# ml4ai/mliis

Hardware: AMD Instinct MI355X
Metric: inner-loop images/sec (EfficientLab-6-3, 224x224, 5-shot) (higher is better)
Workload: dtype f32 (the long-K decoder convs and their filter gradients with every operand split exactly into three bf16 terms on the matrix cores, 6 term products, f32 accumulate: fp32-equivalent products; everything else the fp32 instruction)

## Files before the change

mliis_amd/csrc/mbconv_small.hip:

```cpp
#include "common.hpp"

namespace mliis {

constexpr int kSmThreads = 512;
constexpr int kSmWaves = kSmThreads / 64;
constexpr int kSmMaxPix = 2048;

struct SmallGeom {
  int N, H, W, C, HS, nitems, npix;
};

template <int V>
struct SmV {
  float v[V];
};
#define SMV_FOR _Pragma("unroll") for (int i = 0; i < V; ++i)
template <int V> __device__ __forceinline__ SmV<V> vzero() { SmV<V> r; SMV_FOR r.v[i] = 0.f; return r; }
template <int V> __device__ __forceinline__ SmV<V> vfill(float x) { SmV<V> r; SMV_FOR r.v[i] = x; return r; }
template <int V> __device__ __forceinline__ SmV<V> vadd(SmV<V> a, SmV<V> b) { SMV_FOR a.v[i] += b.v[i]; return a; }
template <int V> __device__ __forceinline__ SmV<V> vsub(SmV<V> a, SmV<V> b) { SMV_FOR a.v[i] -= b.v[i]; return a; }
template <int V> __device__ __forceinline__ SmV<V> vmul(SmV<V> a, SmV<V> b) { SMV_FOR a.v[i] *= b.v[i]; return a; }
template <int V> __device__ __forceinline__ SmV<V> vscale(SmV<V> a, float s) { SMV_FOR a.v[i] *= s; return a; }
template <int V> __device__ __forceinline__ SmV<V> vfma(SmV<V> a, SmV<V> b, SmV<V> c) { SMV_FOR c.v[i] = fmaf(a.v[i], b.v[i], c.v[i]); return c; }
template <int V> __device__ __forceinline__ SmV<V> vswish(SmV<V> a) { SMV_FOR a.v[i] = swish_f(a.v[i]); return a; }
template <int V> __device__ __forceinline__ SmV<V> vswish_grad(SmV<V> a) { SMV_FOR a.v[i] = swish_grad_f(a.v[i]); return a; }
template <int V> __device__ __forceinline__ SmV<V> vxhat(SmV<V> x, SmV<V> m, SmV<V> r) { SMV_FOR x.v[i] = (x.v[i] - m.v[i]) * r.v[i]; return x; }
template <int V> __device__ __forceinline__ SmV<V> vaffine(SmV<V> xh, SmV<V> g, SmV<V> b) { SMV_FOR xh.v[i] = fmaf(xh.v[i], g.v[i], b.v[i]); return xh; }
template <int V> __device__ __forceinline__ SmV<V> vbn_dx(SmV<V> g, SmV<V> xh, SmV<V> a, SmV<V> b, SmV<V> ga, SmV<V> rs) {
  SMV_FOR g.v[i] = ga.v[i] * rs.v[i] * (g.v[i] - a.v[i] - xh.v[i] * b.v[i]);
  return g;
}
template <int V> __device__ __forceinline__ SmV<V> vld(const float* __restrict__ p) { SmV<V> r; SMV_FOR r.v[i] = p[i]; return r; }
template <int V> __device__ __forceinline__ void vst(float* __restrict__ p, SmV<V> a) { SMV_FOR p[i] = a.v[i]; }

template <int V> struct SmSlot { static constexpr int F = V; };
template <int V> __device__ __forceinline__ SmV<V> lds_ld(const float* __restrict__ base, int slot) {
  SmV<V> r;
  if constexpr (V == 2) {
    const float2 t = *reinterpret_cast<const float2*>(base + slot * 2);
    r.v[0] = t.x; r.v[1] = t.y;
  } else {
    const float4 t = *reinterpret_cast<const float4*>(base + slot * 4);
    r.v[0] = t.x; r.v[1] = t.y; r.v[2] = t.z; r.v[V - 1] = t.w;
  }
  return r;
}
template <int V> __device__ __forceinline__ void lds_st(float* __restrict__ base, int slot, SmV<V> a) {
  if constexpr (V == 2) {
    *reinterpret_cast<float2*>(base + slot * 2) = make_float2(a.v[0], a.v[1]);
  } else {
    *reinterpret_cast<float4*>(base + slot * 4) = make_float4(a.v[0], a.v[1], a.v[2], a.v[V - 1]);
  }
}

template <int V> struct SmRun { static constexpr int R = 32 / V; };
template <int V>
__device__ __forceinline__ int sm_channel_group(int C) {
  constexpr int R = SmRun<V>::R;
  const int G = C / V, runs = (G + R - 1) / R;
  const int b = blockIdx.x, xcd = b & 7, j = b >> 3;
  const int run = (j / R) * 8 + xcd, sub = j % R;
  if (run >= runs) return -1;
  const int gq = run * R + sub;
  return gq < G ? gq : -1;
}
static inline int sm_grid(int C, int V) {
  const int R = 32 / V, G = C / V, runs = (G + R - 1) / R;
  return ((runs + 7) / 8) * 8 * R;
}
static inline int sm_group_width(int C, int k, int cus) { return (k == 5 && C % 2 == 0 && C / 2 <= cus) ? 2 : 4; }

template <int CTRL, int ROW_MASK>
__device__ __forceinline__ float sm_dpp_add(float v) {
  return v + __builtin_bit_cast(float, __builtin_amdgcn_update_dpp(0, __builtin_bit_cast(int, v), CTRL, ROW_MASK, 0xF, true));
}
__device__ __forceinline__ float sm_wave_sum63(float v) {
  v = sm_dpp_add<0xB1, 0xF>(v);
  v = sm_dpp_add<0x4E, 0xF>(v);
  v = sm_dpp_add<0x141, 0xF>(v);
  v = sm_dpp_add<0x140, 0xF>(v);
  v = sm_dpp_add<0x142, 0xA>(v);
  v = sm_dpp_add<0x143, 0xC>(v);
  return v;
}
template <int V> __device__ __forceinline__ SmV<V> sm_wave_sum63(SmV<V> a) { SMV_FOR a.v[i] = sm_wave_sum63(a.v[i]); return a; }

__device__ __forceinline__ void sm_lds_barrier() {
  __builtin_amdgcn_fence(__ATOMIC_RELEASE, "workgroup", "local");
  __builtin_amdgcn_s_barrier();
  __builtin_amdgcn_fence(__ATOMIC_ACQUIRE, "workgroup", "local");
}

template <int V>
__device__ __forceinline__ void sm_block_sum2(SmV<V>& a, SmV<V>& b, float* red) {
  const int t = threadIdx.x, lane = t & 63, wave = t >> 6;
  const SmV<V> wa = sm_wave_sum63(a), wb = sm_wave_sum63(b);
  if (lane == 63) {
    SMV_FOR {
      red[(wave * 2 + 0) * 4 + i] = wa.v[i];
      red[(wave * 2 + 1) * 4 + i] = wb.v[i];
    }
  }
  sm_lds_barrier();
  if (t < 8) {
    float sacc = red[t];
#pragma unroll
    for (int w = 1; w < kSmWaves; ++w) sacc += red[w * 8 + t];
    red[kSmWaves * 8 + t] = sacc;
  }
  sm_lds_barrier();
  SMV_FOR {
    a.v[i] = red[kSmWaves * 8 + i];
    b.v[i] = red[kSmWaves * 8 + 4 + i];
  }
}

typedef unsigned sm_u32x4 __attribute__((ext_vector_type(4)));
typedef unsigned sm_u32x2 __attribute__((ext_vector_type(2)));
constexpr unsigned kSmOob = 0xFFFFFFF0u;
__device__ __forceinline__ __amdgpu_buffer_rsrc_t sm_rsrc(const void* p) {
  return __builtin_amdgcn_make_buffer_rsrc(const_cast<void*>(p), 0, 0x80000000u, 0x00020000);
}
template <int V, typename T = float>
__device__ __forceinline__ SmV<V> sm_ld(__amdgpu_buffer_rsrc_t r, unsigned off) {
  SmV<V> o;
  if constexpr (sizeof(T) == 2 && V == 2) {
    const unsigned u = __builtin_amdgcn_raw_buffer_load_b32(r, (int)off, 0, 0);
    o.v[0] = __uint_as_float(u << 16); o.v[1] = __uint_as_float(u & 0xffff0000u);
  } else if constexpr (sizeof(T) == 2) {
    const sm_u32x2 u = __builtin_amdgcn_raw_buffer_load_b64(r, (int)off, 0, 0);
    o.v[0] = __uint_as_float(u.x << 16); o.v[1] = __uint_as_float(u.x & 0xffff0000u);
    o.v[2] = __uint_as_float(u.y << 16); o.v[V - 1] = __uint_as_float(u.y & 0xffff0000u);
  } else if constexpr (V == 2) {
    const sm_u32x2 u = __builtin_amdgcn_raw_buffer_load_b64(r, (int)off, 0, 0);
    o.v[0] = __uint_as_float(u.x); o.v[1] = __uint_as_float(u.y);
  } else {
    const sm_u32x4 u = __builtin_amdgcn_raw_buffer_load_b128(r, (int)off, 0, 0);
    o.v[0] = __uint_as_float(u.x); o.v[1] = __uint_as_float(u.y); o.v[2] = __uint_as_float(u.z); o.v[3] = __uint_as_float(u.w);
  }
  return o;
}
template <int V, typename T = float>
__device__ __forceinline__ void sm_st(__amdgpu_buffer_rsrc_t r, unsigned off, SmV<V> a) {
  if constexpr (sizeof(T) == 2 && V == 2) {
    __builtin_amdgcn_raw_buffer_store_b32(pack_bf16_pair(a.v[0], a.v[1]), r, (int)off, 0, 0);
  } else if constexpr (sizeof(T) == 2) {
    sm_u32x2 u;
    u.x = pack_bf16_pair(a.v[0], a.v[1]); u.y = pack_bf16_pair(a.v[2], a.v[V - 1]);
    __builtin_amdgcn_raw_buffer_store_b64(u, r, (int)off, 0, 0);
  } else if constexpr (V == 2) {
    sm_u32x2 u;
    u.x = __float_as_uint(a.v[0]); u.y = __float_as_uint(a.v[1]);
    __builtin_amdgcn_raw_buffer_store_b64(u, r, (int)off, 0, 0);
  } else {
    sm_u32x4 u;
    u.x = __float_as_uint(a.v[0]); u.y = __float_as_uint(a.v[1]); u.z = __float_as_uint(a.v[2]); u.w = __float_as_uint(a.v[V - 1]);
    __builtin_amdgcn_raw_buffer_store_b128(u, r, (int)off, 0, 0);
  }
}

template <int V, typename T> __device__ __forceinline__ SmV<V> sm_stored(SmV<V> a) {
  if constexpr (sizeof(T) == 2) {
#pragma unroll
    for (int i = 0; i < V; ++i) a.v[i] = bf16_round_f(a.v[i]);
  }
  return a;
}

struct SmStrip {
  bool act;
  int n, h0, w;
  unsigned off0, rstride;
  int H;
  __device__ __forceinline__ unsigned poff(int j) const { return (act && h0 + j < H) ? off0 + (unsigned)j * rstride : kSmOob; }
  unsigned boff0, brow;
  __device__ __forceinline__ unsigned bpoff(int j) const { return (act && h0 + j < H) ? boff0 + (unsigned)j * brow : kSmOob; }
  __device__ __forceinline__ bool ok(int j) const { return act && h0 + j < H; }
};
__device__ __forceinline__ SmStrip sm_strip(const SmallGeom& g, int c, int esize = 4, int V = 4) {
  SmStrip s;
  const int pl = threadIdx.x;
  s.act = pl < g.nitems;
  int w_ = 0, hs = 0, n = 0;
  if (s.act) {
    w_ = pl % g.W;
    const int r = pl / g.W;
    hs = r % g.HS;
    n = r / g.HS;
  }
  s.n = n;
  s.h0 = hs * 4;
  s.w = w_;
  s.H = g.H;
  s.off0 = (unsigned)((((n * g.H + s.h0) * g.W + w_) * g.C + c) * esize);
  s.rstride = (unsigned)(g.W * g.C * esize);
  s.boff0 = (unsigned)((((c / V) * g.npix + (n * g.H + s.h0) * g.W + w_) * V) * esize);
  s.brow = (unsigned)(g.W * V * esize);
  return s;
}

struct SmallFwd {
  const float* z0;
  const float* part0;
  int nblk0;
  const float *gamma0, *beta0;
  float *mean0, *rstd0, *mm0, *mv0;
  const float* w;
  const float *gamma1, *beta1;
  float *mean1, *rstd1, *mm1, *mv1;
  float* a0;
  float* z1;
  float* a1;
  float* s;
  float* z0b;
  int z1_blocked;
  SmallGeom g;
  float eps, one_minus_momentum;
};

template <int K, int V> struct SmTapsInRegs { static constexpr bool value = K == 3 || V <= 2; };

template <int K, int V, typename T = float>
__global__ __launch_bounds__(kSmThreads) void mbconv_dw_fwd_small_k(SmallFwd p) {
  extern __shared__ __attribute__((aligned(16))) float smem[];
  typedef SmV<V> VT;
  constexpr int F = SmSlot<V>::F;
  const SmallGeom g = p.g;
  float* tileA = smem;
  float* wl = tileA + (size_t)g.npix * F;
  float* red = wl + K * K * F;
  float* pool = red + (kSmWaves + 1) * 2 * 4;
  double* fold = reinterpret_cast<double*>(pool + kSmThreads * F);
  float* stat = reinterpret_cast<float*>(fold + 8);
  const int cq = sm_channel_group<V>(g.C);
  if (cq < 0) return;
  const int t = threadIdx.x, lane = t & 63, wave = t >> 6;
  const int c = cq * V;
  const SmStrip st = sm_strip(g, c, (int)sizeof(T), V);
// ... 55 lines not shown
  VT acc[4];
#pragma unroll
  for (int j = 0; j < 4; ++j) acc[j] = vzero<V>();
  if (st.act) {
    const float* imgA = tileA + (size_t)st.n * g.H * g.W * F;
    if constexpr (SmTapsInRegs<K, V>::value) {
      VT wreg[K * K];
#pragma unroll
      for (int i = 0; i < K * K; ++i) wreg[i] = lds_ld<V>(wl, i);
#pragma unroll
      for (int r = 0; r < K + 3; ++r) {
        const int hi = st.h0 - P + r;
        const bool rok = (unsigned)hi < (unsigned)g.H;
        VT row[K];
#pragma unroll
        for (int kx = 0; kx < K; ++kx) {
          const int wi = st.w - P + kx;
          row[kx] = (rok && (unsigned)wi < (unsigned)g.W) ? lds_ld<V>(imgA, hi * g.W + wi) : vzero<V>();
        }
#pragma unroll
        for (int j = 0; j < 4; ++j) {
          const int ky = r - j;
          if (ky >= 0 && ky < K) {
#pragma unroll
            for (int kx = 0; kx < K; ++kx) acc[j] = vfma(row[kx], wreg[ky * K + kx], acc[j]);
          }
        }
        if (K == 5) __builtin_amdgcn_sched_barrier(0);
      }
    } else {
#pragma unroll 1
      for (int r = 0; r < K + 3; ++r) {
        const int hi = st.h0 - P + r;
        const bool rok = (unsigned)hi < (unsigned)g.H;
        VT row[K];
#pragma unroll
        for (int kx = 0; kx < K; ++kx) {
          const int wi = st.w - P + kx;
          row[kx] = (rok && (unsigned)wi < (unsigned)g.W) ? lds_ld<V>(imgA, hi * g.W + wi) : vzero<V>();
        }
#pragma unroll
        for (int j = 0; j < 4; ++j) {
          const int ky = r - j;
          if (ky >= 0 && ky < K) {
#pragma unroll
            for (int kx = 0; kx < K; ++kx) acc[j] = vfma(row[kx], lds_ld<V>(wl, ky * K + kx), acc[j]);
          }
        }
      }
    }
  }
  {
    const __amdgpu_buffer_rsrc_t rz1 = sm_rsrc(p.z1);
#pragma unroll
    for (int j = 0; j < 4; ++j) {
      acc[j] = sm_stored<V, T>(acc[j]);
      sm_st<V, T>(rz1, p.z1_blocked ? st.bpoff(j) : st.poff(j), acc[j]);
    }
  }
  VT s1 = vzero<V>(), s2 = vzero<V>();
#pragma unroll
  for (int j = 0; j < 4; ++j)
    if (st.ok(j)) s1 = vadd(s1, acc[j]);
  sm_block_sum2<V>(s1, s2, red);
  const float inv_n = 1.0f / (float)g.npix;
  const VT m1 = vscale(s1, inv_n);
  VT d2 = vzero<V>(), dummy = vzero<V>();
#pragma unroll
  for (int j = 0; j < 4; ++j)
    if (st.ok(j)) {
      const VT d = vsub(acc[j], m1);
      d2 = vfma(d, d, d2);
    }
  sm_block_sum2<V>(d2, dummy, red);
  const VT var1 = vscale(d2, inv_n);
  VT r1;
  SMV_FOR r1.v[i] = 1.0f / sqrtf(var1.v[i] + p.eps);
  VT a1v[4];
  {
    const VT ga = vld<V>(p.gamma1 + c), be = vld<V>(p.beta1 + c);
    VT ps = vzero<V>();
#pragma unroll
    for (int j = 0; j < 4; ++j) {
      a1v[j] = sm_stored<V, T>(vswish(vaffine(vxhat(acc[j], m1, r1), ga, be)));
      if (st.ok(j)) ps = vadd(ps, a1v[j]);
    }
    lds_st<V>(pool, t, ps);
    const __amdgpu_buffer_rsrc_t ra1 = sm_rsrc(p.a1);
#pragma unroll
    for (int j = 0; j < 4; ++j) sm_st<V, T>(ra1, st.poff(j), a1v[j]);
  }
  sm_lds_barrier();
  {
    const int per = g.HS * g.W;
    for (int img = wave; img < g.N; img += kSmWaves) {
      VT a = vzero<V>();
      for (int i = lane; i < per; i += 64) a = vadd(a, lds_ld<V>(pool, img * per + i));
      a = sm_wave_sum63(a);
      if (lane == 63) vst<V>(p.s + (long long)img * g.C + c, vscale(a, 1.0f / (float)(g.H * g.W)));
    }
  }
  if (t < V) {
    const float mf = stat[t], vf = stat[8 + t];
    p.mean0[c + t] = mf;
    p.rstd0[c + t] = stat[4 + t];
    if (p.mm0 != nullptr) {
      p.mm0[c + t] = mmv0 - (mmv0 - mf) * p.one_minus_momentum;
      p.mv0[c + t] = mvv0 - (mvv0 - vf) * p.one_minus_momentum;
    }
    float m1t = 0.f, r1t = 0.f, v1t = 0.f;
    SMV_FOR if (i == t) {
      m1t = m1.v[i];
      r1t = r1.v[i];
      v1t = var1.v[i];
    }
    p.mean1[c + t] = m1t;
    p.rstd1[c + t] = r1t;
    if (p.mm1 != nullptr) {
      p.mm1[c + t] = mmv1 - (mmv1 - m1t) * p.one_minus_momentum;
      p.mv1[c + t] = mvv1 - (mvv1 - v1t) * p.one_minus_momentum;
    }
  }
}

struct SmallBwd {
  const float* da2;
  const float* gate;
  const float* chan_add;
  const float* z1;
  const float *mean1, *rstd1, *gamma1, *beta1;
  const float* w;
  const float* z0;
  const float *mean0, *rstd0, *gamma0, *beta0;
  float *dgamma1, *dbeta1, *dw, *dgamma0, *dbeta0;
  float* dz0;
  const float* z0b;
  int z1_blocked;
  SmallGeom g;
};

template <int K, int V, typename T = float>
__global__ __launch_bounds__(kSmThreads) void mbconv_dw_bwd_small_k(SmallBwd p) {
  extern __shared__ __attribute__((aligned(16))) float smem[];
  typedef SmV<V> VT;
  constexpr int F = SmSlot<V>::F;
  const SmallGeom g = p.g;
  float* tileA = smem;
  float* tileD = tileA + (size_t)g.npix * F;
  float* wl = tileD + (size_t)g.npix * F;
  float* red = wl + K * K * F;
  float* wred = red + (kSmWaves + 1) * 2 * 4;
  constexpr bool PARK = K == 5 && V == 4;
  float* tileX = wred + kSmWaves * K * K * F;
  const int cq = sm_channel_group<V>(g.C);
  if (cq < 0) return;
  const int t = threadIdx.x, lane = t & 63, wave = t >> 6;
  const int c = cq * V;
  const SmStrip st = sm_strip(g, c, (int)sizeof(T), V);
  const float inv_n = 1.0f / (float)g.npix;
  VT zv[4], dv[4], z0v[4];
  {
    const bool zb = p.z0b != nullptr;
    const __amdgpu_buffer_rsrc_t rz1 = sm_rsrc(p.z1), rd = sm_rsrc(p.da2), rz0 = sm_rsrc(zb ? p.z0b : p.z0);
#pragma unroll
    for (int j = 0; j < 4; ++j) {
      zv[j] = sm_ld<V, T>(rz1, (p.z1_blocked & 1) ? st.bpoff(j) : st.poff(j));
      dv[j] = sm_ld<V, T>(rd, (p.z1_blocked & 2) ? st.bpoff(j) : st.poff(j));
      z0v[j] = sm_ld<V, T>(rz0, zb ? st.bpoff(j) : st.poff(j));
    }
  }
  if (t < K * K) lds_st<V>(wl, t, vld<V>(p.w + (long long)t * g.C + c));
  VT gt = vfill<V>(1.f), ca = vzero<V>();
  if (st.act && p.gate != nullptr) gt = vld<V>(p.gate + (long long)st.n * g.C + c);
  if (st.act && p.chan_add != nullptr) ca = vld<V>(p.chan_add + (long long)st.n * g.C + c);
  const VT m0 = vld<V>(p.mean0 + c), r0_ = vld<V>(p.rstd0 + c), ga0_ = vld<V>(p.gamma0 + c), be0_ = vld<V>(p.beta0 + c);
  {
    const VT m1 = vld<V>(p.mean1 + c), r1 = vld<V>(p.rstd1 + c), ga = vld<V>(p.gamma1 + c), be = vld<V>(p.beta1 + c);
    VT s1 = vzero<V>(), s2 = vzero<V>();
#pragma unroll
    for (int j = 0; j < 4; ++j) {
      const VT xh = vxhat(zv[j], m1, r1);
      VT gg = vmul(vfma(dv[j], gt, ca), vswish_grad(vaffine(xh, ga, be)));
      if (!st.ok(j)) gg = vzero<V>();
      zv[j] = xh;
      dv[j] = gg;
      s1 = vadd(s1, gg);
      s2 = vfma(gg, xh, s2);
    }
    sm_block_sum2<V>(s1, s2, red);
    if (t == 0) {
      vst<V>(p.dbeta1 + c, s1);
      vst<V>(p.dgamma1 + c, s2);
    }
    const VT a = vscale(s1, inv_n), b = vscale(s2, inv_n);
#pragma unroll
    for (int j = 0; j < 4; ++j) {
      const VT d = vbn_dx(dv[j], zv[j], a, b, ga, r1);
      dv[j] = st.ok(j) ? d : vzero<V>();
      if (st.ok(j)) lds_st<V>(tileD, (st.n * g.H + st.h0 + j) * g.W + st.w, d);
    }
  }
#pragma unroll
  for (int j = 0; j < 4; ++j) {
    const VT xh = vxhat(z0v[j], m0, r0_);
    z0v[j] = xh;
    if (st.ok(j)) lds_st<V>(tileA, (st.n * g.H + st.h0 + j) * g.W + st.w, vswish(vaffine(xh, ga0_, be0_)));
    if (PARK && st.ok(j)) lds_st<V>(tileX, (st.n * g.H + st.h0 + j) * g.W + st.w, xh);
  }
  __syncthreads();
  constexpr int P = (K - 1) / 2;
  {
    VT wacc[K * K];
#pragma unroll
    for (int i = 0; i < K * K; ++i) wacc[i] = vzero<V>();
    if (st.act) {
      const float* imgA = tileA + (size_t)st.n * g.H * g.W * F;
#pragma unroll
      for (int r = 0; r < K + 3; ++r) {
        const int hi = st.h0 - P + r;
        const bool rok = (unsigned)hi < (unsigned)g.H;
        VT row[K];
#pragma unroll
        for (int kx = 0; kx < K; ++kx) {
          const int wi = st.w - P + kx;
          row[kx] = (rok && (unsigned)wi < (unsigned)g.W) ? lds_ld<V>(imgA, hi * g.W + wi) : vzero<V>();
        }
#pragma unroll
        for (int j = 0; j < 4; ++j) {
          const int ky = r - j;
          if (ky >= 0 && ky < K) {
#pragma unroll
            for (int kx = 0; kx < K; ++kx) wacc[ky * K + kx] = vfma(row[kx], dv[j], wacc[ky * K + kx]);
          }
        }
        if (K == 5) __builtin_amdgcn_sched_barrier(0);
      }
    }
#pragma unroll
    for (int i = 0; i < K * K; ++i) {
      const VT v = sm_wave_sum63(wacc[i]);
      if (lane == 63) lds_st<V>(wred, wave * (K * K) + i, v);
    }
  }
  __builtin_amdgcn_sched_barrier(0);
  VT acc[4];
#pragma unroll
  for (int j = 0; j < 4; ++j) acc[j] = vzero<V>();
  if (st.act) {
    const float* imgD = tileD + (size_t)st.n * g.H * g.W * F;
    constexpr bool REGS = SmTapsInRegs<K, V>::value;
    VT wreg[REGS ? K * K : 1];
    if constexpr (REGS) {
#pragma unroll
      for (int i = 0; i < K * K; ++i) wreg[i] = lds_ld<V>(wl, i);
    }
    auto body = [&](int r) {
      const int hi = st.h0 - P + r;
      const bool rok = (unsigned)hi < (unsigned)g.H;
      VT row[K];
#pragma unroll
      for (int x = 0; x < K; ++x) {
        const int wi = st.w - P + x;
        row[x] = (rok && (unsigned)wi < (unsigned)g.W) ? lds_ld<V>(imgD, hi * g.W + wi) : vzero<V>();
      }
#pragma unroll
      for (int j = 0; j < 4; ++j) {
        const int ky = (K - 1) - (r - j);
        if (ky >= 0 && ky < K) {
#pragma unroll
          for (int x = 0; x < K; ++x) {
            const VT wv = REGS ? wreg[REGS ? ky * K + (K - 1 - x) : 0] : lds_ld<V>(wl, ky * K + (K - 1 - x));
            acc[j] = vfma(row[x], wv, acc[j]);
          }
        }
      }
    };
    if constexpr (REGS) {
#pragma unroll
      for (int r = 0; r < K + 3; ++r) {
        body(r);
        if (K == 5) __builtin_amdgcn_sched_barrier(0);
      }
    } else {
#pragma unroll 1
      for (int r = 0; r < K + 3; ++r) body(r);
    }
  }
  __syncthreads();
  if (t < K * K) {
    VT v = lds_ld<V>(wred, t);
#pragma unroll
    for (int wv = 1; wv < kSmWaves; ++wv) v = vadd(v, lds_ld<V>(wred, wv * (K * K) + t));
    vst<V>(p.dw + (long long)t * g.C + c, v);
  }
  {
    VT ga0 = ga0_, be0 = be0_, r0 = r0_;
    if constexpr (PARK) {
      const float* pg = p.gamma0 + c;
      const float* pb = p.beta0 + c;
      const float* pr = p.rstd0 + c;
      asm volatile("" : "+v"(pg), "+v"(pb), "+v"(pr));
      ga0 = vld<V>(pg);
      be0 = vld<V>(pb);
      r0 = vld<V>(pr);
#pragma unroll
      for (int j = 0; j < 4; ++j) z0v[j] = st.ok(j) ? lds_ld<V>(tileX, (st.n * g.H + st.h0 + j) * g.W + st.w) : vzero<V>();
    }
    VT s1 = vzero<V>(), s2 = vzero<V>();
#pragma unroll
    for (int j = 0; j < 4; ++j) {
      VT gg = vmul(acc[j], vswish_grad(vaffine(z0v[j], ga0, be0)));
      if (!st.ok(j)) gg = vzero<V>();
      acc[j] = gg;
      s1 = vadd(s1, gg);
      s2 = vfma(gg, z0v[j], s2);
    }
    sm_block_sum2<V>(s1, s2, red);
    if (t == 0) {
      vst<V>(p.dbeta0 + c, s1);
      vst<V>(p.dgamma0 + c, s2);
    }
    const VT a = vscale(s1, inv_n), b = vscale(s2, inv_n);
    const __amdgpu_buffer_rsrc_t rdz = sm_rsrc(p.dz0);
#pragma unroll
    for (int j = 0; j < 4; ++j)
      if (st.ok(j)) sm_st<V, T>(rdz, st.poff(j), vbn_dx(acc[j], z0v[j], a, b, ga0, r0));
  }
}
#undef SMV_FOR

static bool small_geom(int N, int H, int W, int C, int k, int stride, SmallGeom* g) {
  if (N <= 0 || H <= 0 || W <= 0 || C <= 0 || (C & 3) || stride != 1 || (k != 3 && k != 5)) return false;
  const long long npix = (long long)N * H * W;
  const int HS = (H + 3) / 4;
  const long long nitems = (long long)N * HS * W;
  if (npix > kSmMaxPix || nitems > kSmThreads || npix * C * 4 >= (1LL << 31)) return false;
  *g = SmallGeom{N, H, W, C, HS, (int)nitems, (int)npix};
  return true;
}
static size_t small_fwd_lds(const SmallGeom& g, int k) {
  return ((size_t)g.npix + (size_t)k * k + (kSmWaves + 1) * 2 + kSmThreads) * 16 + 8 * 8 + 16 * 4;
}
static size_t small_bwd_lds(const SmallGeom& g, int k) { return ((size_t)g.npix * (k == 5 ? 3 : 2) + (size_t)k * k + (kSmWaves + 1) * 2 + (size_t)kSmWaves * k * k) * 16; }

template <typename Kern>
static int small_attr(Kern kern, size_t lds_max, int* done) {
  if (*done) return MLIIS_OK;
  hipError_t e = hipFuncSetAttribute(reinterpret_cast<const void*>(kern), hipFuncAttributeMaxDynamicSharedMemorySize, (int)lds_max);
  if (e != hipSuccess) return set_error(MLIIS_ERR_LAUNCH, "mbconv_small: cannot reserve %zu bytes of LDS: %s", lds_max, hipGetErrorString(e));
  *done = 1;
  return MLIIS_OK;
}
static int sm_num_cus() {
  static int cus = 0;
  if (cus == 0) {
    int dev = 0;
    hipDeviceProp_t prop;
    cus = (hipGetDevice(&dev) == hipSuccess && hipGetDeviceProperties(&prop, dev) == hipSuccess && prop.multiProcessorCount > 0)
              ? prop.multiProcessorCount : 256;
  }
  return cus;
}
static SmallGeom small_max_geom() { return SmallGeom{1, 1, 1, 4, 1, kSmThreads, kSmMaxPix}; }

template <int K, int V, typename T>
static int small_launch_fwd_t(const SmallFwd& p, int C, size_t lds, hipStream_t stream) {
  static int attr = 0;
  int rc;
  if ((rc = small_attr(mbconv_dw_fwd_small_k<K, V, T>, small_fwd_lds(small_max_geom(), K), &attr))) return rc;
  hipLaunchKernelGGL((mbconv_dw_fwd_small_k<K, V, T>), dim3(sm_grid(C, V)), dim3(kSmThreads), lds, stream, p);
  return MLIIS_OK;
}
template <int K, int V>
static int small_launch_fwd(const SmallFwd& p, int C, size_t lds, int dt, hipStream_t stream) {
  return dt == MLIIS_DT_BF16 ? small_launch_fwd_t<K, V, bf16s>(p, C, lds, stream) : small_launch_fwd_t<K, V, float>(p, C, lds, stream);
}
template <int K, int V, typename T>
static int small_launch_bwd_t(const SmallBwd& p, int C, size_t lds, hipStream_t stream) {
  static int attr = 0;
  int rc;
  if ((rc = small_attr(mbconv_dw_bwd_small_k<K, V, T>, small_bwd_lds(small_max_geom(), K), &attr))) return rc;
  hipLaunchKernelGGL((mbconv_dw_bwd_small_k<K, V, T>), dim3(sm_grid(C, V)), dim3(kSmThreads), lds, stream, p);
  return MLIIS_OK;
}
template <int K, int V>
static int small_launch_bwd(const SmallBwd& p, int C, size_t lds, int dt, hipStream_t stream) {
  return dt == MLIIS_DT_BF16 ? small_launch_bwd_t<K, V, bf16s>(p, C, lds, stream) : small_launch_bwd_t<K, V, float>(p, C, lds, stream);
}

}

using namespace mliis;

extern "C" {

int mliis_mbconv_dw_small_supported(int N, int H, int W, int C, int k, int stride) {
  SmallGeom g;
  return small_geom(N, H, W, C, k, stride, &g) ? 1 : 0;
}

int mliis_mbconv_dw_small_group_width(int C, int k) { return C > 0 ? sm_group_width(C, k, sm_num_cus()) : 0; }

int mliis_mbconv_dw_fwd_small(const float* z0, const float* part0, int nblk0, const float* gamma0, const float* beta0, float* mean0,
                              float* rstd0, float* moving_mean0, float* moving_var0, const float* w, const float* gamma1, const float* beta1,
                              float* mean1, float* rstd1, float* moving_mean1, float* moving_var1, float* a0, float* z1, float* a1, float* s,
                              int N, int H, int W, int C, int k, float eps, float momentum, int group_width, int act_dtype, float* z0_blocked,
                              int z1_blocked, hipStream_t stream) {
  SmallGeom g;
  MLIIS_REQUIRE(small_geom(N, H, W, C, k, 1, &g), MLIIS_ERR_UNSUPPORTED,
                "mbconv_dw_fwd_small: shape N=%d H=%d W=%d C=%d k=%d is not eligible (mliis_mbconv_dw_small_supported)", N, H, W, C, k);
  MLIIS_REQUIRE(z0 && part0 && nblk0 > 0 && gamma0 && beta0 && mean0 && rstd0 && w && gamma1 && beta1 && mean1 && rstd1 && z1 && a1 && s,
                MLIIS_ERR_ARG, "mbconv_dw_fwd_small: null pointer");
  MLIIS_REQUIRE((moving_mean0 == nullptr) == (moving_var0 == nullptr) && (moving_mean1 == nullptr) == (moving_var1 == nullptr), MLIIS_ERR_ARG,
                "mbconv_dw_fwd_small: moving mean / variance come in pairs");
  MLIIS_REQUIRE(aligned16(z0) && aligned16(part0) && aligned16(gamma0) && aligned16(beta0) && aligned16(mean0) && aligned16(rstd0) &&
                    aligned16(w) && aligned16(gamma1) && aligned16(beta1) && aligned16(mean1) && aligned16(rstd1) && aligned16(a0) &&
                    aligned16(z1) && aligned16(a1) && aligned16(s) && aligned16(moving_mean1) && aligned16(moving_var1),
                MLIIS_ERR_ALIGN, "mbconv_dw_fwd_small: pointers must be 16-byte aligned");
  const int V = group_width ? group_width : sm_group_width(C, k, sm_num_cus());
  MLIIS_REQUIRE((V == 2 || V == 4) && C % V == 0, MLIIS_ERR_ARG, "mbconv_dw_fwd_small: group_width %d must be 0, 2 or 4 and divide C = %d", V, C);
  MLIIS_REQUIRE(aligned16(z0_blocked), MLIIS_ERR_ALIGN, "mbconv_dw_fwd_small: z0_blocked must be 16-byte aligned");
  SmallFwd p{z0, part0, nblk0, gamma0, beta0, mean0, rstd0, moving_mean0, moving_var0, w, gamma1, beta1, mean1, rstd1, moving_mean1,
             moving_var1, a0, z1, a1, s, z0_blocked, z1_blocked, g, eps, 1.0f - momentum};
  const size_t lds = small_fwd_lds(g, k);
  int rc;
  MLIIS_REQUIRE(act_dtype == MLIIS_DT_F32 || act_dtype == MLIIS_DT_BF16, MLIIS_ERR_ARG, "mbconv_dw_fwd_small: bad act_dtype");
  if (k == 3) rc = V == 2 ? small_launch_fwd<3, 2>(p, C, lds, act_dtype, stream) : small_launch_fwd<3, 4>(p, C, lds, act_dtype, stream);
  else rc = V == 2 ? small_launch_fwd<5, 2>(p, C, lds, act_dtype, stream) : small_launch_fwd<5, 4>(p, C, lds, act_dtype, stream);
  if (rc) return rc;
  MLIIS_CHECK_LAUNCH("mbconv_dw_fwd_small");
  return MLIIS_OK;
}

int mliis_mbconv_dw_bwd_small(const float* da2, const float* gate, const float* chan_add, const float* z1, const float* mean1,
                              const float* rstd1, const float* gamma1, const float* beta1, const float* w, const float* z0, const float* mean0,
                              const float* rstd0, const float* gamma0, const float* beta0, float* dgamma1, float* dbeta1, float* dw,
                              float* dgamma0, float* dbeta0, float* dz0, int N, int H, int W, int C, int k, int group_width, int act_dtype,
                              const float* z0_blocked, int z1_blocked, hipStream_t stream) {
  SmallGeom g;
  MLIIS_REQUIRE(small_geom(N, H, W, C, k, 1, &g), MLIIS_ERR_UNSUPPORTED,
                "mbconv_dw_bwd_small: shape N=%d H=%d W=%d C=%d k=%d is not eligible (mliis_mbconv_dw_small_supported)", N, H, W, C, k);
  MLIIS_REQUIRE(da2 && z1 && mean1 && rstd1 && gamma1 && beta1 && w && z0 && mean0 && rstd0 && gamma0 && beta0 && dgamma1 && dbeta1 && dw &&
                    dgamma0 && dbeta0 && dz0,
                MLIIS_ERR_ARG, "mbconv_dw_bwd_small: null pointer");
  MLIIS_REQUIRE(aligned16(da2) && aligned16(gate) && aligned16(chan_add) && aligned16(z1) && aligned16(mean1) && aligned16(rstd1) &&
                    aligned16(gamma1) && aligned16(beta1) && aligned16(w) && aligned16(z0) && aligned16(mean0) && aligned16(rstd0) &&
                    aligned16(gamma0) && aligned16(beta0) && aligned16(dgamma1) && aligned16(dbeta1) && aligned16(dw) && aligned16(dgamma0) &&
                    aligned16(dbeta0) && aligned16(dz0),
                MLIIS_ERR_ALIGN, "mbconv_dw_bwd_small: pointers must be 16-byte aligned");
  const int V = group_width ? group_width : sm_group_width(C, k, sm_num_cus());
  MLIIS_REQUIRE((V == 2 || V == 4) && C % V == 0, MLIIS_ERR_ARG, "mbconv_dw_bwd_small: group_width %d must be 0, 2 or 4 and divide C = %d", V, C);
  MLIIS_REQUIRE(aligned16(z0_blocked), MLIIS_ERR_ALIGN, "mbconv_dw_bwd_small: z0_blocked must be 16-byte aligned");
  SmallBwd p{da2, gate, chan_add, z1, mean1, rstd1, gamma1, beta1, w, z0, mean0, rstd0, gamma0, beta0, dgamma1, dbeta1, dw, dgamma0, dbeta0,
             dz0, z0_blocked, z1_blocked, g};
  const size_t lds = small_bwd_lds(g, k);
  int rc;
  MLIIS_REQUIRE(act_dtype == MLIIS_DT_F32 || act_dtype == MLIIS_DT_BF16, MLIIS_ERR_ARG, "mbconv_dw_bwd_small: bad act_dtype");
  if (k == 3) rc = V == 2 ? small_launch_bwd<3, 2>(p, C, lds, act_dtype, stream) : small_launch_bwd<3, 4>(p, C, lds, act_dtype, stream);
  else rc = V == 2 ? small_launch_bwd<5, 2>(p, C, lds, act_dtype, stream) : small_launch_bwd<5, 4>(p, C, lds, act_dtype, stream);
  if (rc) return rc;
  MLIIS_CHECK_LAUNCH("mbconv_dw_bwd_small");
  return MLIIS_OK;
}
}
```

mliis_amd/csrc/se.hip:

```cpp
#include "common.hpp"
#include "se_wgrad.hpp"

namespace mliis {

constexpr int kMaxR = 128;
constexpr int kSeThreads = 1024;

template <int U>
__device__ __forceinline__ float dot_strided(const float* __restrict__ a, int sa, const float* __restrict__ b, long long sb, int n) {
  float acc = 0.f;
  for (int i = 0; i < n; i += U) {
    float x[U], y[U];
#pragma unroll
    for (int u = 0; u < U; ++u) {
      const int k = i + u < n ? i + u : n - 1;
      x[u] = a[(long long)k * sa];
      y[u] = b[(long long)k * sb];
    }
#pragma unroll
    for (int u = 0; u < U; ++u) acc = fmaf(i + u < n ? x[u] : 0.f, y[u], acc);
  }
  return acc;
}

constexpr int kSeFastDot = 24;
template <bool FAST>
__global__ __launch_bounds__(kSeThreads) void se_mlp_fwd_k(const float* __restrict__ s_part, int chunks, float scale,
                                                    float* __restrict__ s_out, const float* __restrict__ w1,
                                                    const float* __restrict__ b1, const float* __restrict__ w2,
                                                    const float* __restrict__ b2, float* __restrict__ hpre,
                                                    float* __restrict__ gate, int C, int R) {
  __shared__ float sh[kMaxR];
  __shared__ float red[kSeThreads];
  __shared__ float red2[8 * kMaxR];
  extern __shared__ float sn[];
  const int n = blockIdx.x, t = threadIdx.x;
  const int CL = kSeThreads / R;
  const int j = t % R, cl = t / R;
  const int cnt = (cl < CL && cl < C) ? (C - cl + CL - 1) / CL : 0;
  float w1v[FAST ? kSeFastDot : 1], w2v[FAST ? 32 : 1], b1v = 0.f, b2v = 0.f;
  if constexpr (FAST) {
    const int cc = t < C ? t : C - 1;
#pragma unroll
    for (int i = 0; i < kSeFastDot; ++i) w1v[i] = w1[(long long)(cl + (i < cnt ? i : 0) * CL < C ? cl + (i < cnt ? i : 0) * CL : 0) * R + j];
#pragma unroll
    for (int k = 0; k < 32; ++k) w2v[k] = w2[(long long)(k < R ? k : R - 1) * C + cc];
    b1v = b1[t < R ? t : 0];
    b2v = b2[cc];
  }
  for (int c = t; c < C; c += kSeThreads) {
    const float* pp = s_part + ((long long)n * chunks) * C + c;
    float a = 0.f;
    for (int k = 0; k < chunks; k += 8) {
      float v[8];
#pragma unroll
      for (int u = 0; u < 8; ++u) v[u] = pp[(long long)(k + u < chunks ? k + u : chunks - 1) * C];
#pragma unroll
      for (int u = 0; u < 8; ++u) a += k + u < chunks ? v[u] : 0.f;
    }
    a *= scale;
    sn[c] = a;
    if (s_out != nullptr) s_out[(long long)n * C + c] = a;
  }
  __syncthreads();
  float part = 0.f;
  if constexpr (FAST) {
#pragma unroll
    for (int i = 0; i < kSeFastDot; ++i) part = fmaf(i < cnt ? sn[cl + i * CL] : 0.f, w1v[i], part);
  } else {
    if (cnt > 0) part = dot_strided<8>(sn + cl, CL, w1 + (long long)cl * R + j, (long long)CL * R, cnt);
  }
  red[t] = part;
  __syncthreads();
  if (t < 8 * R) {
    const int g = t / R;
    float h = 0.f;
    for (int k = g; k < CL; k += 8) h += red[k * R + j];
    red2[g * R + j] = h;
  }
  __syncthreads();
  if (t < R) {
    float h = FAST ? b1v : b1[t];
#pragma unroll
    for (int g = 0; g < 8; ++g) h += red2[g * R + t];
    hpre[(long long)n * R + t] = h;
    sh[t] = swish_f(h);
  }
  __syncthreads();
  if constexpr (FAST) {
    if (t < C) {
      float a = b2v;
#pragma unroll
      for (int k = 0; k < 32; ++k) a = fmaf(k < R ? sh[k] : 0.f, w2v[k], a);
      gate[(long long)n * C + t] = sigmoid_f(a);
    }
    return;
  }
  for (int c = t; c < C; c += kSeThreads) {
    float a = b2[c];
    for (int k = 0; k < R; k += 8) {
      float wv[8];
#pragma unroll
      for (int u = 0; u < 8; ++u) wv[u] = w2[(long long)(k + u < R ? k + u : R - 1) * C + c];
#pragma unroll
      for (int u = 0; u < 8; ++u) a = fmaf(k + u < R ? sh[k + u] : 0.f, wv[u], a);
    }
    gate[(long long)n * C + c] = sigmoid_f(a);
  }
}

template <bool FAST>
__global__ __launch_bounds__(kSeThreads) void se_mlp_bwd_k(const float* __restrict__ dgate, int dgate_groups, int HW,
                                                    const float* __restrict__ gate,
                                                    const float* __restrict__ hpre, const float* __restrict__ w1,
                                                    const float* __restrict__ w1t,
                                                    const float* __restrict__ w2, float* __restrict__ dpre2,
                                                    float* __restrict__ dpre1, float* __restrict__ chan_add, int C, int R,
                                                    float inv_hw, const float* __restrict__ sums, int sums_nblk,
                                                    float* __restrict__ stage1) {
  __shared__ float sd1[kMaxR];
  extern __shared__ float sd2[];
  const int n = blockIdx.x, t = threadIdx.x, lane = t & 63, wave = t >> 6;
  float* d2 = dpre2 + (long long)n * C;
  const int g_lo = dgate_groups > 0 ? (n * HW) / 16 : 0, g_hi = dgate_groups > 0 ? ((n + 1) * HW - 1) / 16 : -1;
  if constexpr (FAST) {
    const int cc = t < C ? t : C - 1;
    const float gte = gate[(long long)n * C + cc];
    float w2v[2][16], w1v[32], hp[2];
#pragma unroll
    for (int r = 0; r < 2; ++r) {
      const int jj = wave + 16 * r < R ? wave + 16 * r : R - 1;
      hp[r] = hpre[(long long)n * R + jj];
#pragma unroll
      for (int u = 0; u < 16; ++u) w2v[r][u] = w2[(long long)jj * C + (lane + 64 * u < C ? lane + 64 * u : C - 1)];
    }
#pragma unroll
    for (int k = 0; k < 32; ++k) {
      const int kk = k < R ? k : R - 1;
      w1v[k] = w1t != nullptr ? w1t[(long long)kk * C + cc] : w1[(long long)cc * R + kk];
    }
    float dg = 0.f;
    if (sums != nullptr) {
      const int G = kSeThreads / C;
      const int g = t / C, c = t - g * C;
      float* scr = sd2 + 5 * C;
      if (g < G) {
        float p[5] = {0.f, 0.f, 0.f, 0.f, 0.f};
        const float* base = sums + ((long long)n * sums_nblk) * 5 * C + c;
        for (int b = g; b < sums_nblk; b += 4 * G) {
          float v[4][5];
#pragma unroll
          for (int u = 0; u < 4; ++u)
#pragma unroll
            for (int k = 0; k < 5; ++k) v[u][k] = base[((long long)(b + u * G < sums_nblk ? b + u * G : b) * 5 + k) * C];
#pragma unroll
          for (int u = 0; u < 4; ++u)
            if (b + u * G < sums_nblk) {
#pragma unroll
              for (int k = 0; k < 5; ++k) p[k] += v[u][k];
            }
        }
#pragma unroll
        for (int k = 0; k < 5; ++k) scr[(g * 5 + k) * C + c] = p[k];
      }
      __syncthreads();
      if (t < C) {
        float p[5] = {0.f, 0.f, 0.f, 0.f, 0.f};
        for (int gg = 0; gg < G; ++gg) {
#pragma unroll
          for (int k = 0; k < 5; ++k) p[k] += scr[(gg * 5 + k) * C + t];
        }
        dg = p[0];
#pragma unroll
        for (int k = 1; k < 5; ++k) sd2[k * C + t] = p[k];
      }
    } else if (dgate_groups > 0) {
      for (int k = g_lo; k <= g_hi; k += 16) {
        float v[16];
#pragma unroll
        for (int u = 0; u < 16; ++u) {
          const int rg = k + u <= g_hi ? k + u : g_hi;
          const int slot = rg * 16 >= n * HW ? 0 : 1;
          v[u] = dgate[((long long)rg * 2 + slot) * C + cc];
        }
#pragma unroll
        for (int u = 0; u < 16; ++u) dg += k + u <= g_hi ? v[u] : 0.f;
      }
    } else {
      dg = dgate[(long long)n * C + cc];
    }
    if (t < C) {
      const float v = dg * gte * (1.f - gte);
      d2[t] = v;
      sd2[t] = v;
    }
    __syncthreads();
#pragma unroll
    for (int r = 0; r < 2; ++r) {
      const int jj = wave + 16 * r;
      if (jj < R) {
        float p = 0.f;
#pragma unroll
        for (int u = 0; u < 16; ++u) p = fmaf(lane + 64 * u < C ? sd2[lane + 64 * u] : 0.f, w2v[r][u], p);
        p = wave_sum(p);
        if (lane == 0) {
          const float d = p * swish_grad_f(hp[r]);
          sd1[jj] = d;
          dpre1[(long long)n * R + jj] = d;
        }
      }
    }
    __syncthreads();
    if (t < C) {
      float a = 0.f;
#pragma unroll
      for (int k = 0; k < 32; ++k) a = fmaf(k < R ? sd1[k] : 0.f, w1v[k], a);
      const float ca = a * inv_hw;
      chan_add[(long long)n * C + t] = ca;
      if (sums != nullptr) {
        stage1[((long long)n * 2 + 0) * C + t] = fmaf(gte, sd2[1 * C + t], ca * sd2[3 * C + t]);
        stage1[((long long)n * 2 + 1) * C + t] = fmaf(gte, sd2[2 * C + t], ca * sd2[4 * C + t]);
      }
    }
    return;
  }
  for (int c = t; c < C; c += kSeThreads) {
    const float g = gate[(long long)n * C + c];
    float dg;
    if (sums != nullptr) {
      float p[5] = {0.f, 0.f, 0.f, 0.f, 0.f};
      const float* base = sums + ((long long)n * sums_nblk) * 5 * C + c;
      for (int b = 0; b < sums_nblk; b += 2) {
        float v[2][5];
#pragma unroll
        for (int u = 0; u < 2; ++u)
#pragma unroll
          for (int k = 0; k < 5; ++k) v[u][k] = base[((long long)(b + u < sums_nblk ? b + u : b) * 5 + k) * C];
#pragma unroll
        for (int u = 0; u < 2; ++u)
          if (b + u < sums_nblk) {
#pragma unroll
            for (int k = 0; k < 5; ++k) p[k] += v[u][k];
          }
      }
      dg = p[0];
#pragma unroll
      for (int k = 1; k < 5; ++k) sd2[k * C + c] = p[k];
    } else if (dgate_groups > 0) {
      dg = 0.f;
      for (int k = g_lo; k <= g_hi; k += 8) {
        float v[8];
#pragma unroll
        for (int u = 0; u < 8; ++u) {
          const int rg = k + u <= g_hi ? k + u : g_hi;
          const int slot = rg * 16 >= n * HW ? 0 : 1;
          v[u] = dgate[((long long)rg * 2 + slot) * C + c];
        }
#pragma unroll
        for (int u = 0; u < 8; ++u) dg += k + u <= g_hi ? v[u] : 0.f;
      }
    } else {
      dg = dgate[(long long)n * C + c];
    }
    const float v = dg * g * (1.f - g);
    d2[c] = v;
    sd2[c] = v;
  }
  __syncthreads();
  for (int jj = wave; jj < R; jj += kSeThreads / 64) {
    const float* wr = w2 + (long long)jj * C;
    float p = 0.f;
    for (int c = lane; c < C; c += 8 * 64) {
      float wv[8];
#pragma unroll
      for (int u = 0; u < 8; ++u) wv[u] = wr[c + u * 64 < C ? c + u * 64 : lane];
#pragma unroll
      for (int u = 0; u < 8; ++u) p = fmaf(c + u * 64 < C ? sd2[c + u * 64] : 0.f, wv[u], p);
    }
    p = wave_sum(p);
    if (lane == 0) {
      const float d = p * swish_grad_f(hpre[(long long)n * R + jj]);
      sd1[jj] = d;
      dpre1[(long long)n * R + jj] = d;
    }
  }
  __syncthreads();
  for (int c = t; c < C; c += kSeThreads) {
    float a = 0.f;
    for (int k = 0; k < R; k += 8) {
      float wv[8];
#pragma unroll
      for (int u = 0; u < 8; ++u) {
        const int kk = k + u < R ? k + u : R - 1;
        wv[u] = w1t != nullptr ? w1t[(long long)kk * C + c] : w1[(long long)c * R + kk];
      }
#pragma unroll
      for (int u = 0; u < 8; ++u) a = fmaf(k + u < R ? sd1[k + u] : 0.f, wv[u], a);
    }
    const float ca = a * inv_hw;
    chan_add[(long long)n * C + c] = ca;
    if (sums != nullptr) {
      const float gt = gate[(long long)n * C + c];
      stage1[((long long)n * 2 + 0) * C + c] = fmaf(gt, sd2[1 * C + c], ca * sd2[3 * C + c]);
      stage1[((long long)n * 2 + 1) * C + c] = fmaf(gt, sd2[2 * C + c], ca * sd2[4 * C + c]);
    }
  }
}

__global__ __launch_bounds__(256) void se_wgrad_k(const float* __restrict__ s, const float* __restrict__ hpre,
                                                  const float* __restrict__ dpre1, const float* __restrict__ dpre2,
                                                  float* __restrict__ dw1, float* __restrict__ db1, float* __restrict__ dw2,
                                                  float* __restrict__ db2, int N, int C, int R) {
  se_wgrad_elem(blockIdx.x * 256 + threadIdx.x, s, hpre, dpre1, dpre2, dw1, db1, dw2, db2, N, C, R);
}

__global__ __launch_bounds__(256) void se_wgrad_batched_k(const long long* __restrict__ desc, int ndesc) {
  se_wgrad_tile(desc, ndesc, blockIdx.x);
}

__global__ __launch_bounds__(256) void chan_affine_k(const float* __restrict__ x, int ldx, const float* __restrict__ S,
                                                     const float* __restrict__ A, float* __restrict__ y, int ldy, long long rows,
                                                     int C, int rows_per_img, int accumulate) {
  const unsigned Q = (unsigned)C >> 2;
  const unsigned total = (unsigned)rows * Q;
  for (unsigned i = blockIdx.x * blockDim.x + threadIdx.x; i < total; i += gridDim.x * blockDim.x) {
    const unsigned ru = i / Q;
    const int c = (int)(i - ru * Q) << 2;
    const long long r = ru;
    const long long n = ru / (unsigned)rows_per_img;
    float* dst = y + r * ldy + c;
    const float4 vx = ld4(x ? x + r * ldx + c : dst);
    const float4 vs = ld4(S ? S + n * C + c : dst);
    const float4 va = ld4(A ? A + n * C + c : dst);
    const float4 vo = ld4(dst);
    float4 v = x ? vx : f4zero();
    if (S) v = f4mul(v, vs);
    if (A) v = f4add(v, va);
    if (accumulate) v = f4add(v, vo);
    st4(dst, v);
  }
}

__global__ __launch_bounds__(256) void chan_split_k(const float* __restrict__ x, int ldx, const float* __restrict__ A, float* __restrict__ y0,
                                                    int ld0, int c0, int acc0, float* __restrict__ y1, int ld1, int acc1, long long rows, int C,
                                                    int rows_per_img) {
  const unsigned Q = (unsigned)C >> 2;
  const unsigned total = (unsigned)rows * Q;
  for (unsigned i = blockIdx.x * blockDim.x + threadIdx.x; i < total; i += gridDim.x * blockDim.x) {
    const unsigned ru = i / Q;
    const int c = (int)(i - ru * Q) << 2;
    const long long r = ru;
    const long long n = ru / (unsigned)rows_per_img;
    const bool first = c < c0;
    float* dst = first ? y0 + r * ld0 + c : y1 + r * ld1 + (c - c0);
    const bool acc = first ? acc0 != 0 : acc1 != 0;
    const float4 vx = ld4(x + r * ldx + c);
    const float4 va = ld4(A ? A + n * C + c : x + r * ldx + c);
    const float4 vo = ld4(dst);
    float4 v = vx;
    if (A) v = f4add(v, va);
    if (acc) v = f4add(v, vo);
    st4(dst, v);
  }
}

}

using namespace mliis;

// ... 96 lines not shown
```

Baseline: 3596.

## Use quad-sum LDS reduction for dw filter grads and skip unused SE weight loads

In the small depthwise backward kernel, the full 64-lane DPP wave reduction of each filter-gradient tap is replaced. Each tap is now reduced within groups of four lanes, the partials are staged in new per-wave LDS, and a second pass spreads the remaining reduction across lanes. The SE MLP forward and backward kernels now load weights and run their dot loops in wave-uniform batches of four (two for w2v in the backward kernel). Batches beyond the actual channel or reduction count, or beyond a wave's owned channels, are skipped. This trades extra LDS space (the backward kernel's reservation grows roughly 17x in its per-wave part) and branching for fewer DPP steps and fewer wasted global loads.

```diff
diff --git a/mliis_amd/csrc/mbconv_small.hip b/mliis_amd/csrc/mbconv_small.hip
--- a/mliis_amd/csrc/mbconv_small.hip
+++ b/mliis_amd/csrc/mbconv_small.hip
@@ -84,6 +84,16 @@
   return v;
 }
 template <int V> __device__ __forceinline__ SmV<V> sm_wave_sum63(SmV<V> a) { SMV_FOR a.v[i] = sm_wave_sum63(a.v[i]); return a; }
+__device__ __forceinline__ float sm_single(float v) {
+  asm("" : "+v"(v));
+  return v;
+}
+__device__ __forceinline__ float sm_quad_sum(float v) {
+  v = sm_single(sm_dpp_add<0xB1, 0xF>(sm_single(v)));
+  v = sm_single(sm_dpp_add<0x4E, 0xF>(v));
+  return v;
+}
+template <int V> __device__ __forceinline__ SmV<V> sm_quad_sum(SmV<V> a) { SMV_FOR a.v[i] = sm_quad_sum(a.v[i]); return a; }
 
 __device__ __forceinline__ void sm_lds_barrier() {
   __builtin_amdgcn_fence(__ATOMIC_RELEASE, "workgroup", "local");
@@ -445,6 +455,7 @@
   float* wred = red + (kSmWaves + 1) * 2 * 4;
   constexpr bool PARK = K == 5 && V == 4;
   float* tileX = wred + kSmWaves * K * K * F;
+  float* qred = tileX + (PARK ? (size_t)g.npix * F : 0);
   const int cq = sm_channel_group<V>(g.C);
   if (cq < 0) return;
   const int t = threadIdx.x, lane = t & 63, wave = t >> 6;
@@ -529,10 +540,24 @@
         if (K == 5) __builtin_amdgcn_sched_barrier(0);
       }
     }
-#pragma unroll
-    for (int i = 0; i < K * K; ++i) {
-      const VT v = sm_wave_sum63(wacc[i]);
-      if (lane == 63) lds_st<V>(wred, wave * (K * K) + i, v);
+    float* qw = qred + (size_t)wave * (K * K * 16) * F;
+#pragma unroll
+    for (int i = 0; i < K * K; ++i) wacc[i] = sm_quad_sum(wacc[i]);
+    if ((lane & 3) == 0) {
+#pragma unroll
+      for (int i = 0; i < K * K; ++i) lds_st<V>(qw, i * 16 + (lane >> 2), wacc[i]);
+    }
+    __builtin_amdgcn_fence(__ATOMIC_RELEASE, "wavefront");
+    __builtin_amdgcn_wave_barrier();
+    __builtin_amdgcn_fence(__ATOMIC_ACQUIRE, "wavefront");
+#pragma unroll
+    for (int it = 0; it < (K * K * 4 + 63) / 64; ++it) {
+      const int item = it * 64 + lane, row = item & 3;
+      const int tap = (item >> 2) < K * K ? (item >> 2) : K * K - 1;
+      const VT q0 = lds_ld<V>(qw, tap * 16 + row * 4 + 0), q1 = lds_ld<V>(qw, tap * 16 + row * 4 + 1);
+      const VT q2 = lds_ld<V>(qw, tap * 16 + row * 4 + 2), q3 = lds_ld<V>(qw, tap * 16 + row * 4 + 3);
+      const VT v = sm_quad_sum(vadd(vadd(q0, q1), vadd(q2, q3)));
+      if (row == 0 && (item >> 2) < K * K) lds_st<V>(wred, wave * (K * K) + tap, v);
     }
   }
   __builtin_amdgcn_sched_barrier(0);
@@ -634,7 +659,7 @@
 static size_t small_fwd_lds(const SmallGeom& g, int k) {
   return ((size_t)g.npix + (size_t)k * k + (kSmWaves + 1) * 2 + kSmThreads) * 16 + 8 * 8 + 16 * 4;
 }
-static size_t small_bwd_lds(const SmallGeom& g, int k) { return ((size_t)g.npix * (k == 5 ? 3 : 2) + (size_t)k * k + (kSmWaves + 1) * 2 + (size_t)kSmWaves * k * k) * 16; }
+static size_t small_bwd_lds(const SmallGeom& g, int k) { return ((size_t)g.npix * (k == 5 ? 3 : 2) + (size_t)k * k + (kSmWaves + 1) * 2 + (size_t)kSmWaves * k * k * (1 + 16)) * 16; }
 
 template <typename Kern>
 static int small_attr(Kern kern, size_t lds_max, int* done) {
diff --git a/mliis_amd/csrc/se.hip b/mliis_amd/csrc/se.hip
--- a/mliis_amd/csrc/se.hip
+++ b/mliis_amd/csrc/se.hip
@@ -24,6 +24,7 @@
 }
 
 constexpr int kSeFastDot = 24;
+constexpr int kSeBatch = 4;
 template <bool FAST>
 __global__ __launch_bounds__(kSeThreads) void se_mlp_fwd_k(const float* __restrict__ s_part, int chunks, float scale,
                                                     float* __restrict__ s_out, const float* __restrict__ w1,
@@ -38,15 +39,32 @@
   const int CL = kSeThreads / R;
   const int j = t % R, cl = t / R;
   const int cnt = (cl < CL && cl < C) ? (C - cl + CL - 1) / CL : 0;
-  float w1v[FAST ? kSeFastDot : 1], w2v[FAST ? 32 : 1], b1v = 0.f, b2v = 0.f;
+  float w1v[FAST ? kSeFastDot : 1] = {}, w2v[FAST ? 32 : 1] = {}, b1v = 0.f, b2v = 0.f;
+  const int wave_u = __builtin_amdgcn_readfirstlane(t >> 6);
+  const int cl_u = (wave_u * 64) / R;
+  const int cnt_u = (cl_u < CL && cl_u < C) ? (C - cl_u + CL - 1) / CL : 0;
+  const bool own_u = wave_u * 64 < C;
   if constexpr (FAST) {
     const int cc = t < C ? t : C - 1;
 #pragma unroll
-    for (int i = 0; i < kSeFastDot; ++i) w1v[i] = w1[(long long)(cl + (i < cnt ? i : 0) * CL < C ? cl + (i < cnt ? i : 0) * CL : 0) * R + j];
-#pragma unroll
-    for (int k = 0; k < 32; ++k) w2v[k] = w2[(long long)(k < R ? k : R - 1) * C + cc];
-    b1v = b1[t < R ? t : 0];
-    b2v = b2[cc];
+    for (int i0 = 0; i0 < kSeFastDot; i0 += kSeBatch) {
+      if (i0 < cnt_u) {
+#pragma unroll
+        for (int i = i0; i < i0 + kSeBatch; ++i)
+          w1v[i] = w1[(long long)(cl + (i < cnt ? i : 0) * CL < C ? cl + (i < cnt ? i : 0) * CL : 0) * R + j];
+      }
+    }
+    if (own_u) {
+#pragma unroll
+      for (int k0 = 0; k0 < 32; k0 += kSeBatch) {
+        if (k0 < R) {
+#pragma unroll
+          for (int k = k0; k < k0 + kSeBatch; ++k) w2v[k] = w2[(long long)(k < R ? k : R - 1) * C + cc];
+        }
+      }
+      b2v = b2[cc];
+    }
+    if (wave_u == 0) b1v = b1[t < R ? t : 0];
   }
   for (int c = t; c < C; c += kSeThreads) {
     const float* pp = s_part + ((long long)n * chunks) * C + c;
@@ -66,7 +84,12 @@
   float part = 0.f;
   if constexpr (FAST) {
 #pragma unroll
-    for (int i = 0; i < kSeFastDot; ++i) part = fmaf(i < cnt ? sn[cl + i * CL] : 0.f, w1v[i], part);
+    for (int i0 = 0; i0 < kSeFastDot; i0 += kSeBatch) {
+      if (i0 < cnt_u) {
+#pragma unroll
+        for (int i = i0; i < i0 + kSeBatch; ++i) part = fmaf(i < cnt ? sn[cl + i * CL] : 0.f, w1v[i], part);
+      }
+    }
   } else {
     if (cnt > 0) part = dot_strided<8>(sn + cl, CL, w1 + (long long)cl * R + j, (long long)CL * R, cnt);
   }
@@ -91,7 +114,12 @@
     if (t < C) {
       float a = b2v;
 #pragma unroll
-      for (int k = 0; k < 32; ++k) a = fmaf(k < R ? sh[k] : 0.f, w2v[k], a);
+      for (int k0 = 0; k0 < 32; k0 += kSeBatch) {
+        if (k0 < R) {
+#pragma unroll
+          for (int k = k0; k < k0 + kSeBatch; ++k) a = fmaf(k < R ? sh[k] : 0.f, w2v[k], a);
+        }
+      }
       gate[(long long)n * C + t] = sigmoid_f(a);
     }
     return;
@@ -126,18 +154,34 @@
   if constexpr (FAST) {
     const int cc = t < C ? t : C - 1;
     const float gte = gate[(long long)n * C + cc];
-    float w2v[2][16], w1v[32], hp[2];
+    const int wave_u = __builtin_amdgcn_readfirstlane(wave);
+    const bool own_u = wave_u * 64 < C;
+    float w2v[2][16] = {}, w1v[32] = {}, hp[2] = {0.f, 0.f};
 #pragma unroll
     for (int r = 0; r < 2; ++r) {
-      const int jj = wave + 16 * r < R ? wave + 16 * r : R - 1;
-      hp[r] = hpre[(long long)n * R + jj];
-#pragma unroll
-      for (int u = 0; u < 16; ++u) w2v[r][u] = w2[(long long)jj * C + (lane + 64 * u < C ? lane + 64 * u : C - 1)];
-    }
-#pragma unroll
-    for (int k = 0; k < 32; ++k) {
-      const int kk = k < R ? k : R - 1;
-      w1v[k] = w1t != nullptr ? w1t[(long long)kk * C + cc] : w1[(long long)cc * R + kk];
+      const int jj = wave_u + 16 * r;
+      if (jj < R) {
+        hp[r] = hpre[(long long)n * R + jj];
+#pragma unroll
+        for (int u0 = 0; u0 < 16; u0 += 2) {
+          if (64 * u0 < C) {
+#pragma unroll
+            for (int u = u0; u < u0 + 2; ++u) w2v[r][u] = w2[(long long)jj * C + (lane + 64 * u < C ? lane + 64 * u : C - 1)];
+          }
+        }
+      }
+    }
+    if (own_u) {
+#pragma unroll
+      for (int k0 = 0; k0 < 32; k0 += kSeBatch) {
+        if (k0 < R) {
+#pragma unroll
+          for (int k = k0; k < k0 + kSeBatch; ++k) {
+            const int kk = k < R ? k : R - 1;
+            w1v[k] = w1t != nullptr ? w1t[(long long)kk * C + cc] : w1[(long long)cc * R + kk];
+          }
+        }
+      }
     }
     float dg = 0.f;
     if (sums != nullptr) {
@@ -175,7 +219,7 @@
         for (int k = 1; k < 5; ++k) sd2[k * C + t] = p[k];
       }
     } else if (dgate_groups > 0) {
-      for (int k = g_lo; k <= g_hi; k += 16) {
+      for (int k = g_lo; own_u && k <= g_hi; k += 16) {
         float v[16];
 #pragma unroll
         for (int u = 0; u < 16; ++u) {
@@ -201,7 +245,12 @@
       if (jj < R) {
         float p = 0.f;
 #pragma unroll
-        for (int u = 0; u < 16; ++u) p = fmaf(lane + 64 * u < C ? sd2[lane + 64 * u] : 0.f, w2v[r][u], p);
+        for (int u0 = 0; u0 < 16; u0 += 2) {
+          if (64 * u0 < C) {
+#pragma unroll
+            for (int u = u0; u < u0 + 2; ++u) p = fmaf(lane + 64 * u < C ? sd2[lane + 64 * u] : 0.f, w2v[r][u], p);
+          }
+        }
         p = wave_sum(p);
         if (lane == 0) {
           const float d = p * swish_grad_f(hp[r]);
@@ -214,7 +263,12 @@
     if (t < C) {
       float a = 0.f;
 #pragma unroll
-      for (int k = 0; k < 32; ++k) a = fmaf(k < R ? sd1[k] : 0.f, w1v[k], a);
+      for (int k0 = 0; k0 < 32; k0 += kSeBatch) {
+        if (k0 < R) {
+#pragma unroll
+          for (int k = k0; k < k0 + kSeBatch; ++k) a = fmaf(k < R ? sd1[k] : 0.f, w1v[k], a);
+        }
+      }
       const float ca = a * inv_hw;
       chan_add[(long long)n * C + t] = ca;
       if (sums != nullptr) {
```

New measurement: 3660, median of 6. +1.8%, better.
